# resibots/limbo

Measured on AMD Instinct MI355X. Metric: GP compute()+log_lik evaluations/sec at N=4096 D=6 fp64, higher is better.
Workload: dtype f64

## Files before the change

limbo_amd/csrc/potrf_tail.hip:

```cpp
#include "potrf_tile.h"
#include <array>
#include <map>
#include <mutex>
#include <vector>
#ifdef DIAG_TIMING
__device__ long long g_tail_ts[64][4];
__device__ long long g_tail_cyc[64][4];
#define TTS(c, i) do { if (threadIdx.x == 0 && (c) < 64) { g_tail_ts[(c)][(i)] = wall_clock64(); g_tail_cyc[(c)][(i)] = clock64(); } } while (0)
__device__ long long g_tail_ts2[64][12];
#define TTS2(x, on, i) do { if ((on) && threadIdx.x == 0 && ((x).R0 - (x).p0) / NB < 64) g_tail_ts2[((x).R0 - (x).p0) / NB][(i)] = wall_clock64(); } while (0)
#else
#define TTS(c, i) do { } while (0)
#define TTS2(x, on, i) do { } while (0)
#endif

struct TailArgs {
    double* A;
    int64_t lda, t0;
    int nt, nb;
    int nfull;
    int rhs_rows;
    double* Xt;
    int* info;
    double *LP, *SP, *LPn, *SPn;
    int spin_limit;
    const int* order;
    const double* Xg;
    int64_t ldx, Ns;
    const double* Om;
    int64_t ldom;
    double* Al;
    int64_t ldal;
    int P;
};
#define TAIL_LDS_DOUBLES (4 * NB * PS)
static_assert(TAIL_LDS_DOUBLES >= NB * XS + 3 * NB * PS && TAIL_LDS_DOUBLES * 8 <= 160 * 1024, "k_tail LDS carve");
static __device__ __forceinline__ int tail_tile_id(int nb, int b, int c) { return c * nb - (c * (c - 1)) / 2 + (b - c); }

static __device__ __forceinline__ void tail_gen_tile(const TailArgs& a, const KParams* __restrict__ kp, int64_t I, int64_t J0,
                                                     double (&out)[8])
{
    if (I >= a.Ns) {
        const double* om = a.Om + (I - a.Ns) * a.ldom;
#pragma unroll
        for (int it = 0; it < 8; ++it)
            out[it] = om[J0 + 2 * it];
        return;
    }
    double z[8];
#pragma unroll
    for (int it = 0; it < 8; ++it)
        z[it] = 0.0;
    const int D = kp->D;
    for (int d = 0; d < D; ++d) {
        const double* xr = a.Xg + (int64_t)d * a.ldx;
        const double xi = xr[I], ie = kp->inv_ell[d];
#pragma unroll
        for (int it = 0; it < 8; ++it) {
            const double q = (xi - xr[J0 + 2 * it]) * ie;
            z[it] = fma(q, q, z[it]);
        }
    }
    const int kind = kp->kind;
    const double sf2 = kp->sf2, da = kp->diag_add;
#pragma unroll
    for (int it = 0; it < 8; ++it)
        out[it] = kfun_fast_rt(kind, z[it], sf2) + (I == J0 + 2 * it ? da : 0.0);
}

#define CH_T 10240
#define CH_X11 (CH_T + NB * PS)
#define CH_LD (CH_X11 + 32 * 34)
#define CH_D 0
#define CH_AUX (NB * XS)
#define CH_YS (CH_AUX + 1096)
#define CH_X22 (CH_AUX + 1096 + DIAG_XW_DOUBLES)
static_assert(CH_X22 + 32 * 34 <= CH_T && CH_YS + 32 * PS <= CH_X22 && CH_LD + 32 * 34 <= 4 * NB * PS, "chain workgroup LDS carve");

template <int KLEN>
static __device__ __forceinline__ void syrk40(const double* __restrict__ Aop, int ak0, int wave, int lane, double (&acc)[5])
{
    const int r16 = lane & 15, kq = lane >> 4, c4 = lane & 3;
    const int j1 = wave, j2 = 15 - wave;
    if (wave < 4) {
#pragma unroll
        for (int ks = 0; ks < KLEN; ks += 4) {
            const double* row = Aop + (ak0 + ks + kq) * PS;
            const double a0 = row[r16], a1 = row[16 + r16], a2 = row[32 + r16], a3 = row[48 + r16];
            const double b1 = row[4 * j1 + c4], b2 = row[4 * j2 + c4];
            acc[0] = mfma4(a0, b1, acc[0]);
            acc[1] = mfma4(a1, b1, acc[1]);
            acc[2] = mfma4(a2, b1, acc[2]);
            acc[3] = mfma4(a3, b1, acc[3]);
            acc[4] = mfma4(a3, b2, acc[4]);
        }
    }
    else {
#pragma unroll
        for (int ks = 0; ks < KLEN; ks += 4) {
            const double* row = Aop + (ak0 + ks + kq) * PS;
            const double a1 = row[16 + r16], a2 = row[32 + r16], a3 = row[48 + r16];
            const double b1 = row[4 * j1 + c4], b2 = row[4 * j2 + c4];
            acc[0] = mfma4(a1, b1, acc[0]);
            acc[1] = mfma4(a2, b1, acc[1]);
            acc[2] = mfma4(a3, b1, acc[2]);
            acc[3] = mfma4(a2, b2, acc[3]);
            acc[4] = mfma4(a3, b2, acc[4]);
        }
    }
}
static __host__ __device__ __forceinline__ int tri_solve_cols(int wave)
{
    const int hq = wave >> 1;
    return hq == 0 ? 0 : (hq == 1 ? 8 : (hq == 2 ? 24 : 16));
}
static __device__ __forceinline__ void tri_solve32(const double* __restrict__ Aop, int ak0, const double* __restrict__ X, int wm,
                                                   int hn, int lane, double (&y)[2][2])
{
    const int ar = wm + (lane & 15), bc = hn + (lane & 3), kq = lane >> 4;
#pragma unroll
    for (int ks = 0; ks < 32; ks += 4) {
        if (ks >= hn + 8)
            break;
        double af[2], bf[2];
#pragma unroll
        for (int m = 0; m < 2; ++m)
            af[m] = Aop[(ak0 + ks + kq) * PS + ar + 16 * m];
#pragma unroll
        for (int n = 0; n < 2; ++n)
            bf[n] = X[(bc + 4 * n) * 34 + ks + kq];
#pragma unroll
        for (int n = 0; n < 2; ++n)
#pragma unroll
            for (int m = 0; m < 2; ++m)
                y[m][n] = mfma4(af[m], bf[n], y[m][n]);
    }
}

template <int NW, int STRIDE = 512>
static __device__ __forceinline__ void chain_watch(const unsigned long long* __restrict__ p, unsigned long long (&b)[NW], int spin_limit,
                                                   int* __restrict__ info)
{
    static_assert(NW == 2 || NW == 4, "written out: the words stay in registers");
    const unsigned long long SENT = ~0ull;
    int spins = 0;
    if constexpr (NW == 4) {
        while (b[0] == SENT || b[1] == SENT || b[2] == SENT || b[3] == SENT) {
            if (++spins > spin_limit) {
                info[2] = 1;
                break;
            }
            if (b[0] == SENT) b[0] = __hip_atomic_load(p, __ATOMIC_RELAXED, __HIP_MEMORY_SCOPE_AGENT);
            if (b[1] == SENT) b[1] = __hip_atomic_load(p + STRIDE, __ATOMIC_RELAXED, __HIP_MEMORY_SCOPE_AGENT);
            if (b[2] == SENT) b[2] = __hip_atomic_load(p + 2 * STRIDE, __ATOMIC_RELAXED, __HIP_MEMORY_SCOPE_AGENT);
            if (b[3] == SENT) b[3] = __hip_atomic_load(p + 3 * STRIDE, __ATOMIC_RELAXED, __HIP_MEMORY_SCOPE_AGENT);
        }
    }
    else {
        while (b[0] == SENT || b[1] == SENT) {
            if (++spins > spin_limit) {
                info[2] = 1;
                break;
            }
            if (b[0] == SENT) b[0] = __hip_atomic_load(p, __ATOMIC_RELAXED, __HIP_MEMORY_SCOPE_AGENT);
            if (b[1] == SENT) b[1] = __hip_atomic_load(p + STRIDE, __ATOMIC_RELAXED, __HIP_MEMORY_SCOPE_AGENT);
        }
    }
    asm volatile("" ::: "memory");
}
static __device__ __forceinline__ void chain_watch2(const unsigned long long* __restrict__ pa, unsigned long long (&a)[4],
                                                    const unsigned long long* __restrict__ pb, unsigned long long (&b)[4], int spin_limit,
                                                    int* __restrict__ info)
{
    const unsigned long long SENT = ~0ull;
    constexpr int STRIDE = 8 * NB;
    int spins = 0;
    while (a[0] == SENT || a[1] == SENT || a[2] == SENT || a[3] == SENT || b[0] == SENT || b[1] == SENT || b[2] == SENT || b[3] == SENT) {
        if (++spins > spin_limit) {
            info[2] = 1;
            break;
        }
        if (a[0] == SENT) a[0] = __hip_atomic_load(pa, __ATOMIC_RELAXED, __HIP_MEMORY_SCOPE_AGENT);
        if (a[1] == SENT) a[1] = __hip_atomic_load(pa + STRIDE, __ATOMIC_RELAXED, __HIP_MEMORY_SCOPE_AGENT);
        if (a[2] == SENT) a[2] = __hip_atomic_load(pa + 2 * STRIDE, __ATOMIC_RELAXED, __HIP_MEMORY_SCOPE_AGENT);
        if (a[3] == SENT) a[3] = __hip_atomic_load(pa + 3 * STRIDE, __ATOMIC_RELAXED, __HIP_MEMORY_SCOPE_AGENT);
        if (b[0] == SENT) b[0] = __hip_atomic_load(pb, __ATOMIC_RELAXED, __HIP_MEMORY_SCOPE_AGENT);
        if (b[1] == SENT) b[1] = __hip_atomic_load(pb + STRIDE, __ATOMIC_RELAXED, __HIP_MEMORY_SCOPE_AGENT);
        if (b[2] == SENT) b[2] = __hip_atomic_load(pb + 2 * STRIDE, __ATOMIC_RELAXED, __HIP_MEMORY_SCOPE_AGENT);
        if (b[3] == SENT) b[3] = __hip_atomic_load(pb + 3 * STRIDE, __ATOMIC_RELAXED, __HIP_MEMORY_SCOPE_AGENT);
    }
    asm volatile("" ::: "memory");
}
static __host__ __device__ __forceinline__ void syrk40_units(int wave, int q, int& i, int& j)
{
    if (wave < 4) {
        i = q < 4 ? q : 3;
        j = q < 4 ? wave : 15 - wave;
    }
    else {
        i = q < 3 ? q + 1 : q - 1;
        j = q < 3 ? wave : 15 - wave;
    }
}
static __device__ __forceinline__ void syrk40_load_neg(const double* __restrict__ Dl, int wave, int lane, double (&acc)[5])
{
    const int drow = 4 * ((lane >> 2) & 3) + (lane >> 4), dcol = lane & 3;
#pragma unroll
    for (int q = 0; q < 5; ++q) {
        int i, j;
        syrk40_units(wave, q, i, j);
        acc[q] = -Dl[(16 * i + drow) * XS + 4 * j + dcol];
    }
}
static __device__ __forceinline__ void syrk40_store_neg(double* __restrict__ Dl, int wave, int lane, const double (&acc)[5])
{
    const int drow = 4 * ((lane >> 2) & 3) + (lane >> 4), dcol = lane & 3;
#pragma unroll
    for (int q = 0; q < 5; ++q) {
        int i, j;
        syrk40_units(wave, q, i, j);
        Dl[(16 * i + drow) * XS + 4 * j + dcol] = -acc[q];
    }
}

static __device__ __forceinline__ void tail_chain_updates_and_crossing(const TailArgs& a, const P256& x, double* __restrict__ lds,
                                                                       const int c, const double (&cl)[8], const double (&cv)[8])
{
    const int lane = threadIdx.x & 63, wave = __builtin_amdgcn_readfirstlane(threadIdx.x >> 6);
    const int wm = (wave & 1) * 32, wn = (wave >> 1) * 16;
    const int hn = tri_solve_cols(wave);
    const int crow = wm + (lane & 31), ccol = wn + (lane >> 5);
    const int drow = 4 * ((lane >> 2) & 3) + (lane >> 4), dcol = lane & 3;
    double* const T = lds + CH_T;
    double* const X11 = lds + CH_X11;
    double* const Ld = lds + CH_LD;
    double* const Dl = lds + CH_D;
    double* const Ys = lds + CH_YS;
    double* const X22 = lds + CH_X22;
    const double* Sq = a.SP + (int64_t)(c - 1) * 3072;
    double* pub = a.LP + (int64_t)tail_tile_id(a.nb, c, c - 1) * (NB * NB);
    const unsigned long long* Sp = reinterpret_cast<const unsigned long long*>(Sq) + threadIdx.x;
    double a2v[5];
#pragma unroll
    for (int it = 0; it < 8; ++it)
        lds[crow * XS + ccol + 2 * it] = cv[it];
    __syncthreads();
    syrk40_load_neg(lds, wave, lane, a2v);
    __syncthreads();
    unsigned long long xb[4];
    if (c > 1) {
        PolledTile pa, pb;
        pa.issue(a.LP + (int64_t)tail_tile_id(a.nb, c, 0) * (NB * NB));
        pb.issue(a.LP + (int64_t)tail_tile_id(a.nb, c - 1, 0) * (NB * NB));
        double a2l[2][4] = {{0.0, 0.0, 0.0, 0.0}, {0.0, 0.0, 0.0, 0.0}};
#pragma unroll 1
        for (int s = 0; s < c - 2; ++s) {
            double* const opA = lds + ((c - 2 - s) & 1) * (2 * NB * PS);
            double* const opB = opA + NB * PS;
            pa.finish(a.LP + (int64_t)tail_tile_id(a.nb, c, s) * (NB * NB), x.spin_limit, x.info);
            pa.store(opA);
            pb.finish(a.LP + (int64_t)tail_tile_id(a.nb, c - 1, s) * (NB * NB), x.spin_limit, x.info);
            pb.store(opB);
            pa.issue(a.LP + (int64_t)tail_tile_id(a.nb, c, s + 1) * (NB * NB));
            pb.issue(a.LP + (int64_t)tail_tile_id(a.nb, c - 1, s + 1) * (NB * NB));
            __syncthreads();
            mm64<false>(opA, opB, wm, wn, lane, a2l);
            syrk40<NB>(opA, 0, wave, lane, a2v);
        }
        double* const opA = lds;
        double* const opB = lds + NB * PS;
        {
            const int i = threadIdx.x & 63, kk0 = threadIdx.x >> 6;
            const unsigned long long* ga = reinterpret_cast<const unsigned long long*>(a.LP + (int64_t)tail_tile_id(a.nb, c, c - 2) * (NB * NB)) + i + kk0 * NB;
            const unsigned long long* gb = reinterpret_cast<const unsigned long long*>(a.LP + (int64_t)tail_tile_id(a.nb, c - 1, c - 2) * (NB * NB)) + i + kk0 * NB;
            unsigned long long ha[4] = {pa.b[0], pa.b[1], pa.b[2], pa.b[3]}, hb[4] = {pb.b[0], pb.b[1], pb.b[2], pb.b[3]};
            chain_watch2(ga, ha, gb, hb, x.spin_limit, x.info);
            TTS2(x, true, 8);
#pragma unroll
            for (int q = 0; q < 4; ++q) {
                opA[(kk0 + 8 * q) * PS + i] = __longlong_as_double((long long)ha[q]);
                opB[(kk0 + 8 * q) * PS + i] = __longlong_as_double((long long)hb[q]);
            }
            __syncthreads();
#pragma unroll
            for (int it = 0; it < 8; ++it)
                T[(ccol + 2 * it) * PS + crow] = cl[it];
            mmk<false, 32, 4>(opA, 0, opB, 0, wm, wn, lane, a2l);
            syrk40<32>(opA, 0, wave, lane, a2v);
            unsigned long long ka[4] = {pa.b[4], pa.b[5], pa.b[6], pa.b[7]}, kb[4] = {pb.b[4], pb.b[5], pb.b[6], pb.b[7]};
            chain_watch2(ga + 32 * NB, ka, gb + 32 * NB, kb, x.spin_limit, x.info);
            TTS2(x, true, 9);
#pragma unroll
            for (int q = 0; q < 4; ++q) {
                opA[(32 + kk0 + 8 * q) * PS + i] = __longlong_as_double((long long)ka[q]);
                opB[(32 + kk0 + 8 * q) * PS + i] = __longlong_as_double((long long)kb[q]);
            }
            __syncthreads();
            TTS2(x, true, 10);
            mmk<false, 32, 4>(opA, 32, opB, 32, wm, wn, lane, a2l);
            syrk40<32>(opA, 32, wave, lane, a2v);
#pragma unroll
            for (int q = 0; q < 4; ++q)
                xb[q] = __hip_atomic_load(Sp + 512 * q, __ATOMIC_RELAXED, __HIP_MEMORY_SCOPE_AGENT);
        }
#pragma unroll
        for (int m = 0; m < 2; ++m)
#pragma unroll
            for (int n = 0; n < 4; ++n) {
                double* t = T + (wn + 4 * n + dcol) * PS + wm + 16 * m + drow;
                *t = *t - a2l[m][n];
            }
    }
    else {
#pragma unroll
        for (int it = 0; it < 8; ++it)
            T[(ccol + 2 * it) * PS + crow] = cl[it];
#pragma unroll
        for (int q = 0; q < 4; ++q)
            xb[q] = __hip_atomic_load(Sp + 512 * q, __ATOMIC_RELAXED, POLL_FIRST_SCOPE);
    }
    TTS(c, 0);
    {
        chain_watch<4>(Sp, xb, x.spin_limit, x.info);
        TTS2(x, true, 0);
#pragma unroll
        for (int q = 0; q < 2; ++q) {
            const int e = threadIdx.x + 512 * q;
            X11[(e >> 5) * 34 + (e & 31)] = __longlong_as_double((long long)xb[q]);
            Ld[(e & 31) * 34 + (e >> 5)] = __longlong_as_double((long long)xb[2 + q]);
        }
    }
    __syncthreads();
    diag_flow_init(reinterpret_cast<DiagSync*>(lds + CH_AUX + DIAG_LTB + NB));
    double y1[2][2] = {{0.0, 0.0}, {0.0, 0.0}};
    tri_solve32(T, 0, X11, wm, hn, lane, y1);
#pragma unroll
    for (int m = 0; m < 2; ++m)
#pragma unroll
        for (int n = 0; n < 2; ++n)
            Ys[(hn + 4 * n + dcol) * PS + wm + 16 * m + drow] = y1[m][n];
    __syncthreads();
    TTS2(x, true, 6);
    double u[2][2] = {{0.0, 0.0}, {0.0, 0.0}};
    mmk<true, 32, 2, 34>(Ys, 0, Ld, 0, wm, hn, lane, u);
#pragma unroll
    for (int m = 0; m < 2; ++m)
#pragma unroll
        for (int n = 0; n < 2; ++n) {
            double* t = T + (32 + hn + 4 * n + dcol) * PS + wm + 16 * m + drow;
            *t = *t - u[m][n];
            T[(hn + 4 * n + dcol) * PS + wm + 16 * m + drow] = y1[m][n];
        }
    {
        const int i = threadIdx.x & 63, kk0 = threadIdx.x >> 6;
#pragma unroll
        for (int q = 0; q < 4; ++q) {
            const int col = kk0 + 8 * q;
            __hip_atomic_store(pub + i + NB * col, Ys[col * PS + i], __ATOMIC_RELAXED, __HIP_MEMORY_SCOPE_AGENT);
        }
    }
    TTS2(x, true, 7);
    unsigned long long xc[2];
    xc[0] = __hip_atomic_load(Sp + 2048, __ATOMIC_RELAXED, __HIP_MEMORY_SCOPE_AGENT);
    xc[1] = __hip_atomic_load(Sp + 2048 + 512, __ATOMIC_RELAXED, __HIP_MEMORY_SCOPE_AGENT);
    syrk40<32>(Ys, 0, wave, lane, a2v);
    TTS2(x, true, 1);
    {
        chain_watch<2>(Sp + 2048, xc, x.spin_limit, x.info);
        TTS2(x, true, 2);
        const int e0 = threadIdx.x, e1 = threadIdx.x + 512;
        X22[(e0 >> 5) * 34 + (e0 & 31)] = __longlong_as_double((long long)xc[0]);
        X22[(e1 >> 5) * 34 + (e1 & 31)] = __longlong_as_double((long long)xc[1]);
    }
    __syncthreads();
    TTS2(x, true, 3);
    double y2[2][2] = {{0.0, 0.0}, {0.0, 0.0}};
    tri_solve32(T, 32, X22, wm, hn, lane, y2);
#pragma unroll
    for (int m = 0; m < 2; ++m)
#pragma unroll
        for (int n = 0; n < 2; ++n)
            Ys[(hn + 4 * n + dcol) * PS + wm + 16 * m + drow] = y2[m][n];
    __syncthreads();
    TTS2(x, true, 4);
    syrk40<32>(Ys, 0, wave, lane, a2v);
    syrk40_store_neg(Dl, wave, lane, a2v);
    {
        const int i = threadIdx.x & 63, kk0 = threadIdx.x >> 6;
#pragma unroll
        for (int q = 0; q < 4; ++q) {
            const int col = kk0 + 8 * q;
            __hip_atomic_store(pub + i + NB * (32 + col), Ys[col * PS + i], __ATOMIC_RELAXED, __HIP_MEMORY_SCOPE_AGENT);
        }
    }
#pragma unroll
    for (int m = 0; m < 2; ++m)
#pragma unroll
        for (int n = 0; n < 2; ++n)
            T[(32 + hn + 4 * n + dcol) * PS + wm + 16 * m + drow] = y2[m][n];
    TTS2(x, true, 5);
}

static __device__ __forceinline__ void tail_tile_solve(const P256& x, double* __restrict__ lds, const double (&own)[8],
                                                       const double* __restrict__ Sq, double* __restrict__ pub, const bool near)
{
    const int lane = threadIdx.x & 63, wave = __builtin_amdgcn_readfirstlane(threadIdx.x >> 6);
    const int wm = (wave & 1) * 32, wn = (wave >> 1) * 16;
    const int hn = tri_solve_cols(wave);
    const int crow = wm + (lane & 31), ccol = wn + (lane >> 5);
    const int drow = 4 * ((lane >> 2) & 3) + (lane >> 4), dcol = lane & 3;
    double* const T = lds + CH_T;
    double* const X11 = lds + CH_X11;
    double* const Ld = lds + CH_LD;
    double* const Ys = lds + CH_YS;
    double* const X22 = lds + CH_X22;
    const unsigned long long SENT = ~0ull;
    const unsigned long long* Sp = reinterpret_cast<const unsigned long long*>(Sq) + threadIdx.x;
#pragma unroll
    for (int it = 0; it < 8; ++it)
        T[(ccol + 2 * it) * PS + crow] = own[it];
    {
        unsigned long long xb[4];
#pragma unroll
        for (int q = 0; q < 4; ++q)
            xb[q] = __hip_atomic_load(Sp + 512 * q, __ATOMIC_RELAXED, POLL_FIRST_SCOPE);
        if (near)
            chain_watch<4>(Sp, xb, x.spin_limit, x.info);
        else {
            int spins = 0;
            while (xb[0] == SENT || xb[1] == SENT || xb[2] == SENT || xb[3] == SENT) {
                if (++spins > x.spin_limit) {
                    x.info[2] = 1;
                    break;
                }
                poll_one(Sq + 1023, x.spin_limit, x.info);
                poll_one(Sq + 1024 + 32 * 31, x.spin_limit, x.info);
#pragma unroll
                for (int q = 0; q < 4; ++q)
                    if (xb[q] == SENT)
                        xb[q] = __hip_atomic_load(Sp + 512 * q, __ATOMIC_RELAXED, __HIP_MEMORY_SCOPE_AGENT);
            }
        }
#pragma unroll
        for (int q = 0; q < 2; ++q) {
            const int e = threadIdx.x + 512 * q;
            X11[(e >> 5) * 34 + (e & 31)] = __longlong_as_double((long long)xb[q]);
            Ld[(e & 31) * 34 + (e >> 5)] = __longlong_as_double((long long)xb[2 + q]);
        }
    }
    __syncthreads();
    double y1[2][2] = {{0.0, 0.0}, {0.0, 0.0}};
    tri_solve32(T, 0, X11, wm, hn, lane, y1);
#pragma unroll
    for (int m = 0; m < 2; ++m)
#pragma unroll
        for (int n = 0; n < 2; ++n)
            Ys[(hn + 4 * n + dcol) * PS + wm + 16 * m + drow] = y1[m][n];
    __syncthreads();
    double u[2][2] = {{0.0, 0.0}, {0.0, 0.0}};
    mmk<true, 32, 2, 34>(Ys, 0, Ld, 0, wm, hn, lane, u);
#pragma unroll
    for (int m = 0; m < 2; ++m)
#pragma unroll
        for (int n = 0; n < 2; ++n) {
            double* t = T + (32 + hn + 4 * n + dcol) * PS + wm + 16 * m + drow;
            *t = *t - u[m][n];
            T[(hn + 4 * n + dcol) * PS + wm + 16 * m + drow] = y1[m][n];
        }
    {
        const int i = threadIdx.x & 63, kk0 = threadIdx.x >> 6;
#pragma unroll
        for (int q = 0; q < 4; ++q) {
            const int col = kk0 + 8 * q;
            __hip_atomic_store(pub + i + NB * col, Ys[col * PS + i], __ATOMIC_RELAXED, __HIP_MEMORY_SCOPE_AGENT);
        }
    }
    {
        unsigned long long xc[2];
        xc[0] = __hip_atomic_load(Sp + 2048, __ATOMIC_RELAXED, POLL_FIRST_SCOPE);
        xc[1] = __hip_atomic_load(Sp + 2048 + 512, __ATOMIC_RELAXED, POLL_FIRST_SCOPE);
        if (near)
            chain_watch<2>(Sp + 2048, xc, x.spin_limit, x.info);
        else {
            int spins = 0;
            while (xc[0] == SENT || xc[1] == SENT) {
                if (++spins > x.spin_limit) {
                    x.info[2] = 1;
                    break;
                }
                poll_one(Sq + 2048 + 1023, x.spin_limit, x.info);
                if (xc[0] == SENT)
                    xc[0] = __hip_atomic_load(Sp + 2048, __ATOMIC_RELAXED, __HIP_MEMORY_SCOPE_AGENT);
                if (xc[1] == SENT)
                    xc[1] = __hip_atomic_load(Sp + 2048 + 512, __ATOMIC_RELAXED, __HIP_MEMORY_SCOPE_AGENT);
            }
        }
        const int e0 = threadIdx.x, e1 = threadIdx.x + 512;
        X22[(e0 >> 5) * 34 + (e0 & 31)] = __longlong_as_double((long long)xc[0]);
        X22[(e1 >> 5) * 34 + (e1 & 31)] = __longlong_as_double((long long)xc[1]);
    }
    __syncthreads();
    double y2[2][2] = {{0.0, 0.0}, {0.0, 0.0}};
    tri_solve32(T, 32, X22, wm, hn, lane, y2);
#pragma unroll
    for (int m = 0; m < 2; ++m)
#pragma unroll
        for (int n = 0; n < 2; ++n)
            Ys[(hn + 4 * n + dcol) * PS + wm + 16 * m + drow] = y2[m][n];
    __syncthreads();
    {
        const int i = threadIdx.x & 63, kk0 = threadIdx.x >> 6;
#pragma unroll
        for (int q = 0; q < 4; ++q) {
            const int col = kk0 + 8 * q;
            __hip_atomic_store(pub + i + NB * (32 + col), Ys[col * PS + i], __ATOMIC_RELAXED, __HIP_MEMORY_SCOPE_AGENT);
        }
    }
#pragma unroll
    for (int m = 0; m < 2; ++m)
#pragma unroll
        for (int n = 0; n < 2; ++n)
            T[(32 + hn + 4 * n + dcol) * PS + wm + 16 * m + drow] = y2[m][n];
    __syncthreads();
}

static __device__ __forceinline__ void tail_body(const TailArgs& a, const int wgid, double* __restrict__ lds,
                                                 const KParams* __restrict__ kp = nullptr)
{
    const int lane = threadIdx.x & 63, wave = __builtin_amdgcn_readfirstlane(threadIdx.x >> 6);
    const int wm = (wave & 1) * 32, wn = (wave >> 1) * 16;
    const int crow = wm + (lane & 31), ccol = wn + (lane >> 5);
    int c = 0, b;
    if (a.order) {
        b = __builtin_amdgcn_readfirstlane(a.order[2 * wgid]);
        c = __builtin_amdgcn_readfirstlane(a.order[2 * wgid + 1]);
    }
    else {
        int id = wgid, colh = a.nb;
        while (id >= colh) {
            id -= colh;
            ++c;
            --colh;
        }
        b = c + id;
    }
    const int slot = tail_tile_id(a.nb, b, c);
    const bool mute = a.spin_limit < 0;
    P256 x;
    x.A = a.A;
    x.lda = a.lda;
    x.p0 = a.t0;
    x.R0 = a.t0 + (int64_t)NB * b;
    x.Xt = a.Xt;
    x.info = a.info;
    x.mute = mute;
    x.spin_limit = mute ? -a.spin_limit : a.spin_limit;
    x.nrows = b < a.nfull ? NB : a.rhs_rows;
    x.want_d = false;
    x.Bx = lds;
    x.T0 = lds + NB * XS;
    x.T1 = x.T0 + NB * PS;
    x.T2 = x.T1 + NB * PS;
    x.S22 = a.SP;
    x.HP = a.LP;
    double* const myslot = a.LP + (int64_t)slot * (NB * NB);
    {
        unsigned long long* nx = reinterpret_cast<unsigned long long*>(a.LPn + (int64_t)slot * (NB * NB));
#pragma unroll
        for (int q = 0; q < 8; ++q)
            nx[threadIdx.x + 512 * q] = ~0ull;
        if (b == c) {
            unsigned long long* ns = reinterpret_cast<unsigned long long*>(a.SPn + (int64_t)c * 3072);
#pragma unroll
            for (int q = 0; q < 6; ++q)
                ns[threadIdx.x + 512 * q] = ~0ull;
        }
    }
    if (b == c + 1 && b < a.nt)
        return;
    const int crc = crow < x.nrows ? crow : x.nrows - 1;
    double cv[8];
    if (kp) {
        tail_gen_tile(a, kp, x.R0 + crc, a.t0 + (int64_t)NB * c + ccol, cv);
        if (a.Al && b >= a.nfull && threadIdx.x < NB)
            for (int p = 0; p < a.P; ++p)
                reinterpret_cast<unsigned long long*>(a.Al)[a.t0 + (int64_t)NB * c + threadIdx.x + (int64_t)p * a.ldal] = ~0ull;
    }
    else {
#pragma unroll
        for (int it = 0; it < 8; ++it)
            cv[it] = a.A[x.R0 + crc + (a.t0 + (int64_t)NB * c + ccol + 2 * it) * a.lda];
    }
    if (b == c) {
        double* const Dl = lds + CH_D;
        double* const Ltb = lds + CH_AUX;
        double* const invd = Ltb + DIAG_LTB;
        DiagSync* const sy = reinterpret_cast<DiagSync*>(invd + NB);
        if (c > 0) {
            double cl[8];
            if (kp)
                tail_gen_tile(a, kp, x.R0 + crow, a.t0 + (int64_t)NB * (c - 1) + ccol, cl);
            else {
#pragma unroll
                for (int it = 0; it < 8; ++it)
                    cl[it] = a.A[x.R0 + crow + (a.t0 + (int64_t)NB * (c - 1) + ccol + 2 * it) * a.lda];
            }
            tail_chain_updates_and_crossing(a, x, lds, c, cl, cv);
            TTS(c, 1);
        }
        else {
#pragma unroll
            for (int it = 0; it < 8; ++it)
                Dl[crow * XS + ccol + 2 * it] = cv[it];
            diag_flow_init(sy);
        }
        __syncthreads();
        DiagEarly ea;
        ea.mute = mute;
        ea.S = a.SP + (int64_t)c * 3072;
        TTS(c, 2);
        diag_flow(Dl, Ltb, invd, sy, a.A + x.R0 + x.R0 * a.lda, a.lda, a.Xt + (int64_t)c * (NB * NB), a.info, x.R0, wave, lane,
                  invd + NB + 8, &ea);
        TTS(c, 3);
        if (c > 0) {
            __syncthreads();
            const int i = threadIdx.x & 63, kk0 = threadIdx.x >> 6;
            double* Ag = a.A + x.R0 + (a.t0 + (int64_t)NB * (c - 1)) * a.lda;
            const double* T = lds + CH_T;
#pragma unroll
            for (int q = 0; q < 8; ++q) {
                const int col = kk0 + 8 * q;
                Ag[i + (int64_t)col * a.lda] = T[col * PS + i];
            }
        }
        return;
    }
    PolledTile pa, pb;
    if (c > 0) {
        pa.issue(a.LP + (int64_t)tail_tile_id(a.nb, b, 0) * (NB * NB));
        pb.issue(a.LP + (int64_t)tail_tile_id(a.nb, c, 0) * (NB * NB));
    }
    double a2[2][4] = {{0.0, 0.0, 0.0, 0.0}, {0.0, 0.0, 0.0, 0.0}};
#pragma unroll 1
    for (int s = 0; s < c; ++s) {
        double* const opA = lds + (s & 1) * (2 * NB * PS);
        double* const opB = opA + NB * PS;
        pa.finish(a.LP + (int64_t)tail_tile_id(a.nb, b, s) * (NB * NB), x.spin_limit, x.info);
        pa.store(opA);
        pb.finish(a.LP + (int64_t)tail_tile_id(a.nb, c, s) * (NB * NB), x.spin_limit, x.info);
        pb.store(opB);
        if (s + 1 < c) {
            pa.issue(a.LP + (int64_t)tail_tile_id(a.nb, b, s + 1) * (NB * NB));
            pb.issue(a.LP + (int64_t)tail_tile_id(a.nb, c, s + 1) * (NB * NB));
        }
        __syncthreads();
        mm64<false>(opA, opB, wm, wn, lane, a2);
    }
    if (c > 0) {
        double a2r[8];
        wave_tile_to_rows(a2, a2r, lane);
#pragma unroll
        for (int it = 0; it < 8; ++it)
            cv[it] -= a2r[it];
        __syncthreads();
    }
    tail_tile_solve(x, lds, cv, a.SP + (int64_t)c * 3072, myslot, b - c <= 3);
    {
        const int i = threadIdx.x & 63, kk0 = threadIdx.x >> 6;
        double* Ag = a.A + x.R0 + (a.t0 + (int64_t)NB * c) * a.lda;
        const double* T = lds + CH_T;
        if (i < x.nrows) {
#pragma unroll
            for (int q = 0; q < 8; ++q) {
                const int col = kk0 + 8 * q;
                Ag[i + (int64_t)col * a.lda] = T[col * PS + i];
            }
        }
    }
}

__global__ __launch_bounds__(512) void k_tail(TailArgs a)
{
    __shared__ __attribute__((aligned(16))) double lds[TAIL_LDS_DOUBLES];
    tail_body(a, (int)blockIdx.x, lds);
}
__global__ __launch_bounds__(512) void k_tail_g(TailArgs a, KParams kp)
{
    __shared__ __attribute__((aligned(16))) double lds[TAIL_LDS_DOUBLES];
    tail_body(a, (int)blockIdx.x, lds, &kp);
}
__global__ __launch_bounds__(512) void k_tail_b(TailArgs a, const BatchTab* __restrict__ bt)
{
    __shared__ __attribute__((aligned(16))) double lds[TAIL_LDS_DOUBLES];
    const int G = bt->G, gp = (int)blockIdx.x % G;
    a.A = bt_rebase(bt, gp, a.A);
    a.Xt = bt_rebase(bt, gp, a.Xt);
    a.info = bt_rebase(bt, gp, a.info);
    a.LP = bt_rebase(bt, gp, a.LP);
    a.SP = bt_rebase(bt, gp, a.SP);
    a.LPn = bt_rebase(bt, gp, a.LPn);
    a.SPn = bt_rebase(bt, gp, a.SPn);
    if (a.Xg) {
        a.Xg = bt_rebase(bt, gp, a.Xg);
        a.Om = bt_rebase(bt, gp, a.Om);
        a.Al = bt_rebase(bt, gp, a.Al);
    }
    tail_body(a, (int)blockIdx.x / G, lds, a.Xg ? &bt->kp[gp] : nullptr);
}

__global__ __launch_bounds__(256) void k_ragged_partial(const double* __restrict__ A, int64_t ld, int m, int n, int64_t k, int kc,
                                                        double* __restrict__ part)
{
    __shared__ __attribute__((aligned(16))) double As[32][NB];
    const int li = threadIdx.x & 63, lk = threadIdx.x >> 6;
    const int ti = threadIdx.x & 15, tj = threadIdx.x >> 4;
    const int64_t k0 = (int64_t)blockIdx.x * kc, k1 = k0 + kc < k ? k0 + kc : k;
    double acc[4][4];
#pragma unroll
    for (int r = 0; r < 4; ++r)
#pragma unroll
        for (int c = 0; c < 4; ++c)
            acc[r][c] = 0.0;
    double nx[8];
    auto fetch = [&](int64_t kb) {
#pragma unroll
        for (int q = 0; q < 8; ++q) {
            const int kk = lk + 4 * q;
            nx[q] = (kb + kk < k1 && li < m) ? A[li + (kb + kk) * ld] : 0.0;
        }
    };
    fetch(k0);
    for (int64_t kb = k0; kb < k1; kb += 32) {
        __syncthreads();
#pragma unroll
        for (int q = 0; q < 8; ++q)
            As[lk + 4 * q][li] = nx[q];
        if (kb + 32 < k1)
            fetch(kb + 32);
        __syncthreads();
#pragma unroll 8
        for (int kk = 0; kk < 32; ++kk) {
            double a[4], b[4];
#pragma unroll
            for (int r = 0; r < 4; ++r) {
                a[r] = As[kk][4 * ti + r];
                b[r] = As[kk][4 * tj + r];
            }
#pragma unroll
            for (int r = 0; r < 4; ++r)
#pragma unroll
                for (int c = 0; c < 4; ++c)
                    acc[r][c] = fma(a[r], b[c], acc[r][c]);
        }
    }
    double* out = part + (int64_t)blockIdx.x * (NB * NB);
#pragma unroll
    for (int c = 0; c < 4; ++c)
#pragma unroll
        for (int r = 0; r < 4; ++r)
            out[4 * ti + r + NB * (4 * tj + c)] = acc[r][c];
}
#define RAGGED_MAX_G 32
__global__ __launch_bounds__(256) void k_ragged_fold(double* __restrict__ C, int64_t ldc, int m, int n, int G, const double* __restrict__ part)
{
    const int i = threadIdx.x & 63, j = 4 * (int)blockIdx.x + (threadIdx.x >> 6);
    if (i >= m || j >= n || i < j)
        return;
    double v[RAGGED_MAX_G];
#pragma unroll
    for (int g = 0; g < RAGGED_MAX_G; ++g)
        v[g] = g < G ? part[(int64_t)g * (NB * NB) + i + NB * j] : 0.0;
    double sum = 0.0;
#pragma unroll
    for (int g = 0; g < RAGGED_MAX_G; ++g)
        sum += v[g];
    C[i + (int64_t)j * ldc] -= sum;
}
int ragged_split(int64_t k, int64_t scratch_doubles, int* kc_out)
{
    if (k < 256 || scratch_doubles < 2 * NB * NB)
        return 0;
    int64_t G = k / 64;
    G = G > RAGGED_MAX_G ? RAGGED_MAX_G : G;
    G = G > scratch_doubles / (NB * NB) ? scratch_doubles / (NB * NB) : G;
    const int64_t kc = ((k + G - 1) / G + 31) / 32 * 32;
    G = (k + kc - 1) / kc;
    *kc_out = (int)kc;
    return (int)G;
}
__global__ __launch_bounds__(DIAG_THREADS) void k_ragged_finish(double* __restrict__ C, int64_t ldc, int jb, int P, int G,
                                                                const double* __restrict__ part, double* __restrict__ Lscr,
                                                                double* __restrict__ Xt, int* __restrict__ info, int64_t goff)
{
    __shared__ __attribute__((aligned(16))) double Ls[NB * XS];
    __shared__ __attribute__((aligned(16))) double Ltb[DIAG_LTB];
    __shared__ __attribute__((aligned(16))) double invd[NB];
    __shared__ DiagSync sy;
    __shared__ __attribute__((aligned(16))) double Xw[DIAG_XW_DOUBLES];
    __shared__ double Rr[NB * 65];
    const int lane = threadIdx.x & 63, w = __builtin_amdgcn_readfirstlane(threadIdx.x >> 6);
    const int m = jb + P;
    for (int e = threadIdx.x; e < NB * 65; e += DIAG_THREADS)
        Rr[e] = 0.0;
    for (int e = threadIdx.x; e < NB * NB; e += DIAG_THREADS)
        Ls[(e & 63) * XS + (e >> 6)] = (e & 63) == (e >> 6) ? 1.0 : 0.0;
    __syncthreads();
#pragma unroll 1
    for (int e0 = 0; e0 < NB * jb; e0 += 2 * DIAG_THREADS) {
        double v[2][RAGGED_MAX_G], c0[2];
#pragma unroll
        for (int u = 0; u < 2; ++u) {
            int e = e0 + u * DIAG_THREADS + (int)threadIdx.x;
            e = e < NB * jb ? e : NB * jb - 1;
            const int i = e & 63, j = e >> 6;
#pragma unroll
            for (int g = 0; g < RAGGED_MAX_G; ++g)
                v[u][g] = part[(int64_t)(g < G ? g : G - 1) * (NB * NB) + e];
            c0[u] = C[(i < m ? i : m - 1) + (int64_t)j * ldc];
        }
#pragma unroll
        for (int u = 0; u < 2; ++u) {
            const int e = e0 + u * DIAG_THREADS + (int)threadIdx.x;
            const int i = e & 63, j = e >> 6;
            double sum = 0.0;
#pragma unroll
            for (int g = 0; g < RAGGED_MAX_G; ++g)
                sum += g < G ? v[u][g] : 0.0;
            const double val = c0[u] - sum;
            if (e < NB * jb && i < m && i >= j) {
                if (i < jb)
                    Ls[i * XS + j] = val;
                else
                    Rr[(i - jb) * 65 + j] = val;
            }
        }
    }
    diag_flow_init(&sy);
    __syncthreads();
    diag_flow(Ls, Ltb, invd, &sy, Lscr, NB, Xt, info, goff, w, lane, Xw);
    asm volatile("s_waitcnt vmcnt(0)" ::: "memory");
    __syncthreads();
    for (int e = threadIdx.x; e < NB * NB; e += DIAG_THREADS) {
        const int i = e & 63, j = e >> 6;
        if (i < jb && j <= i)
            C[i + (int64_t)j * ldc] = __hip_atomic_load(Lscr + e, __ATOMIC_RELAXED, __HIP_MEMORY_SCOPE_AGENT);
    }
    if (P > 0) {
        for (int e = threadIdx.x; e < NB * NB; e += DIAG_THREADS)
            Ls[(e >> 6) * XS + (e & 63)] = __hip_atomic_load(Xt + e, __ATOMIC_RELAXED, __HIP_MEMORY_SCOPE_AGENT);
        __syncthreads();
        for (int e = threadIdx.x; e < P * NB; e += DIAG_THREADS) {
            const int c = e & 63, p = e >> 6;
            if (c < jb) {
                double z = 0.0;
                for (int k = 0; k <= c; ++k)
                    z = fma(Rr[p * 65 + k], Ls[c * XS + k], z);
                C[jb + p + (int64_t)c * ldc] = z;
            }
        }
    }
}
bool launch_ragged_finish(hipStream_t s, double* C, int64_t ldc, const double* A, int64_t ld, int64_t jb, int64_t P, int64_t k,
                          double* scratch, int64_t scratch_doubles, double* Xt, int* info, int64_t goff)
{
    const int64_t m = jb + P;
    if (g_batch.bt || g_batch.G != 1 || jb < 1 || jb >= NB || P < 0 || m > NB || !scratch || scratch_doubles < 3 * NB * NB)
        return false;
    int kc = 0;
    const int G = ragged_split(k, scratch_doubles - NB * NB, &kc);
    if (G < 2)
        return false;
    GPE_LAUNCH(k_ragged_partial, dim3((unsigned)G), dim3(256), 0, s, A, ld, (int)m, (int)jb, k, kc, scratch);
    GPE_LAUNCH(k_ragged_finish, dim3(1), dim3(DIAG_THREADS), 0, s, C, ldc, (int)jb, (int)P, G, (const double*)scratch,
               scratch + (int64_t)G * (NB * NB), Xt, info, goff);
    return true;
}
bool launch_ragged_update(hipStream_t s, double* C, int64_t ldc, const double* A, int64_t ld, int64_t m, int64_t n, int64_t k,
                          double* scratch, int64_t scratch_doubles)
{
    if (g_batch.bt || g_batch.G != 1 || m < 1 || m > NB || n < 1 || n > NB || !scratch)
        return false;
    int kc = 0;
    const int G = ragged_split(k, scratch_doubles, &kc);
    if (G < 2)
        return false;
    GPE_LAUNCH(k_ragged_partial, dim3((unsigned)G), dim3(256), 0, s, A, ld, (int)m, (int)n, k, kc, scratch);
    GPE_LAUNCH(k_ragged_fold, dim3(NB / 4), dim3(256), 0, s, C, ldc, (int)m, (int)n, G, (const double*)scratch);
    return true;
}

#define TAIL_DLEAD 4
#define TAIL_DLEAD_MAX_BLOCKED 16
static bool build_tail_order(int nt, int nb, int W, int lag, std::vector<int>& flat, int dlead = 0)
{
    struct T {
        int key, c, b;
    };
    std::vector<T> ts;
    for (int c = 0; c < nt; ++c)
        for (int b = c; b < nb; ++b) {
            int k;
            if (b == c)
                k = 2 * c - 3 - 2 * dlead;
            else if (b >= nt)
                k = 2 * (c + std::max(lag, 0));
            else if (b == c + 1)
                k = 2 * c;
            else
                k = 2 * (W > 0 ? std::max(c, b - W) : c);
            ts.push_back(T{k, c, b});
        }
    std::stable_sort(ts.begin(), ts.end(), [](const T& x, const T& y) {
        if (x.key != y.key)
            return x.key < y.key;
        if (x.c != y.c)
            return x.c < y.c;
        return x.b < y.b;
    });
    auto tid = [&](int b, int c) { return c * nb - (c * (c - 1)) / 2 + (b - c); };
    std::vector<int> pos(ts.size());
    for (size_t i = 0; i < ts.size(); ++i)
        pos[tid(ts[i].b, ts[i].c)] = (int)i;
    auto dpos = [&](int c) { return pos[tid(c, c)]; };
    auto owner = [&](int b, int s) { return (b == s + 1 && b < nt) ? dpos(b) : pos[tid(b, s)]; };
    bool legal = true;
    std::vector<int> blocked(ts.size() + 1, 0);
    for (const T& t : ts) {
        const int me = pos[tid(t.b, t.c)];
        if (t.b == t.c) {
            int last = -1;
            for (int s2 = 0; s2 < t.c - 1; ++s2)
                last = std::max(last, std::max(owner(t.c, s2), owner(t.c - 1, s2)));
            if (last > me) {
                if (dlead <= 0)
                    legal = false;
                ++blocked[(size_t)me + 1];
                --blocked[(size_t)last + 1];
            }
            if (t.c > 0)
                legal = legal && dpos(t.c - 1) < me;
        }
        else if (!(t.b == t.c + 1 && t.b < nt)) {
            for (int s2 = 0; s2 < t.c && legal; ++s2)
                legal = owner(t.b, s2) < me && owner(t.c, s2) < me;
            legal = legal && dpos(t.c) < me;
        }
        if (!legal)
            break;
    }
    for (size_t q = 1, run = 0; q < blocked.size() && legal; ++q) {
        run += blocked[q];
        legal = (int)run <= TAIL_DLEAD_MAX_BLOCKED;
    }
    flat.assign(2 * ts.size(), 0);
    for (size_t i = 0; i < ts.size(); ++i) {
        flat[2 * i] = ts[i].b;
        flat[2 * i + 1] = ts[i].c;
    }
    return legal;
}
static const int* tail_order(int nt, int nb, int dlead, int lag)
{
    const int W = 0;
    if (dlead <= 0 && lag <= 0)
        return nullptr;
    static std::mutex mu;
    static std::map<std::array<int, 6>, int*> cache;
    int dev = 0;
    (void)hipGetDevice(&dev);
    const std::array<int, 6> key{dev, nt, nb, dlead, lag, 0};
    std::lock_guard<std::mutex> lk(mu);
    auto it = cache.find(key);
    if (it != cache.end())
        return it->second;
    std::vector<int> flat;
    int* d = nullptr;
    if (build_tail_order(nt, nb, W, lag, flat, dlead) || (dlead > 0 && build_tail_order(nt, nb, W, lag, flat, 0))) {
        if (hipMalloc(&d, sizeof(int) * flat.size()) != hipSuccess || hipMemcpy(d, flat.data(), sizeof(int) * flat.size(), hipMemcpyHostToDevice) != hipSuccess)
            d = nullptr;
    }
    else
        fprintf(stderr, "gpe: tail_order(%d, %d, lead %d, lag %d) violates a dependency — column-by-column order used\n", nt, nb, dlead, lag);
    cache[key] = d;
    return d;
}
void debug_chain_split(int wave, int* units10, int* cols)
{
    for (int q = 0; q < 5; ++q)
        syrk40_units(wave, q, units10[2 * q], units10[2 * q + 1]);
    *cols = tri_solve_cols(wave);
}
int debug_tail_order(int nt, int nb, int lag, int pair)
{
    if (pair)
        return -1;
    if (nt < 1 || nb < nt || nb > 4096)
        return -1;
    std::vector<int> flat;
    if (!build_tail_order(nt, nb, 0, lag, flat, 0))
        return 0;
    if (!build_tail_order(nt, nb, 0, lag, flat, TAIL_DLEAD))
        return 0;
    std::vector<char> seen((size_t)nt * nb, 0);
    size_t n = 0;
    for (size_t i = 0; i + 1 < flat.size(); i += 2) {
        const int b = flat[i], c = flat[i + 1];
        if (c < 0 || c >= nt || b < c || b >= nb || seen[(size_t)c * nb + b])
            return 0;
        seen[(size_t)c * nb + b] = 1;
        ++n;
    }
    return n == (size_t)(nt * nb - nt * (nt - 1) / 2) ? 1 : 0;
}

void launch_tail(hipStream_t s, double* A, int64_t lda, int64_t t0, int64_t t1, int64_t N64, int64_t M, double* Xt_all, int* info,
                 double* buf_cur, double* buf_next, const TailGen* gen)
{
    TailArgs a{};
    a.A = A;
    a.lda = lda;
    a.t0 = t0;
    a.nt = (int)((t1 - t0) / NB);
    a.nfull = (int)((N64 - t0) / NB);
    a.rhs_rows = (int)(M - N64);
    a.nb = a.nfull + (a.rhs_rows > 0 ? 1 : 0);
    a.Xt = Xt_all + (t0 / NB) * (NB * NB);
    a.info = info;
    a.SP = buf_cur;
    a.LP = buf_cur + (int64_t)a.nt * 3072;
    a.SPn = buf_next;
    a.LPn = buf_next + (int64_t)a.nt * 3072;
    a.spin_limit = flow_spin_limit();
    static const int ord_lag = (int)env_int("GPE_TAIL_LAG", 3);
    a.order = tail_order(a.nt, a.nb, g_batch.bt ? 0 : TAIL_DLEAD, ord_lag);
    const int64_t tiles = tail_tiles(a.nt, a.nb);
    if (gen) {
        a.Xg = gen->Xg;
        a.ldx = gen->ldx;
        a.Ns = gen->Ns;
        a.Om = gen->Om;
        a.ldom = gen->ldom;
        a.Al = gen->Al;
        a.ldal = gen->ldal;
        a.P = gen->P;
    }
    FlowGate gate(s);
    if (g_batch.bt)
        GPE_LAUNCH(k_tail_b, dim3((unsigned)(tiles * g_batch.G)), dim3(512), 0, s, a, g_batch.bt);
    else if (gen)
        GPE_LAUNCH(k_tail_g, dim3((unsigned)tiles), dim3(512), 0, s, a, *gen->kp);
    else
        GPE_LAUNCH(k_tail, dim3((unsigned)tiles), dim3(512), 0, s, a);
}

#ifdef DIAG_TIMING
void dump_tail_timing(int nt)
{
    long long h[64][4];
    hipMemcpyFromSymbol(h, HIP_SYMBOL(g_tail_ts), sizeof(h));
    const long long t0 = h[0][2];
    printf("k_tail, the diagonal workgroups (us after the first one starts factoring): column | earlier updates done | its left tile solved, block complete | factoring | panel wave done\n");
    for (int c = 0; c < nt && c < 64; ++c)
        printf("  %2d | %7.2f | %7.2f | %7.2f | %7.2f   (step %5.2f)\n", c, c ? (h[c][0] - t0) * 0.01 : 0.0, c ? (h[c][1] - t0) * 0.01 : 0.0,
               (h[c][2] - t0) * 0.01, (h[c][3] - t0) * 0.01, c ? (h[c][2] - h[c - 1][2]) * 0.01 : 0.0);
    long long cy[64][4];
    hipMemcpyFromSymbol(cy, HIP_SYMBOL(g_tail_cyc), sizeof(cy));
    printf("  factoring -> panel wave done, per column: us | shader-clock cycles | MHz\n   ");
    for (int c = 0; c < nt && c < 64; ++c)
        printf(" %d: %.2f %lld %.0f |", c, (h[c][3] - h[c][2]) * 0.01, cy[c][3] - cy[c][2], (cy[c][3] - cy[c][2]) / ((h[c][3] - h[c][2]) * 0.01));
    printf("\n");
    long long g[64][12];
    hipMemcpyFromSymbol(g, HIP_SYMBOL(g_tail_ts2), sizeof(g));
    printf("  between two blocks, us after the panel wave of column c-1 is through: X11/L21 seen | phase A done | X22 seen | X22 in LDS | Y2 written | second half product done | block complete | factoring\n");
    for (int c = 1; c < nt && c < 64; ++c) {
        const long long p = h[c - 1][3];
        printf("  %2d | %6.2f | %6.2f | %6.2f | %6.2f | %6.2f | %6.2f | %6.2f | %6.2f   (updates done %6.2f; inside phase A: Y1 in LDS %6.2f, T2 updated + first half out %6.2f)\n", c, (g[c][0] - p) * 0.01, (g[c][1] - p) * 0.01, (g[c][2] - p) * 0.01,
               (g[c][3] - p) * 0.01, (g[c][4] - p) * 0.01, (g[c][5] - p) * 0.01, (h[c][1] - p) * 0.01, (h[c][2] - p) * 0.01, (h[c][0] - p) * 0.01,
               (g[c][6] - p) * 0.01, (g[c][7] - p) * 0.01);
        if (c >= 2)
            printf("       the last update step: first halves of L(c, c-2), L(c-1, c-2) seen %6.2f | second halves seen %6.2f | in LDS %6.2f\n",
                   (g[c][8] - p) * 0.01, (g[c][9] - p) * 0.01, (g[c][10] - p) * 0.01);
    }
}
#endif
```

Measured before the change: 948.9.

## Split tail block's first X11 wait into halves to overlap solve with polling

The diagonal-tile solve in the tail kernel no longer waits for all four published chunks (both X11 halves and L21) at once. It waits for the first X11 half, solves it on the first four waves and starts the syrk product on those rows, then waits for the remaining chunks and solves the second half. The syrk product is split into two 16-row pieces to match, and the final syrk is moved after the second-half publish stores so consumers see data earlier. This adds extra barriers and a variable-arity chain_watch in exchange for overlapping computation with cross-workgroup polling latency.

```diff
diff --git a/limbo_amd/csrc/potrf_tail.hip b/limbo_amd/csrc/potrf_tail.hip
--- a/limbo_amd/csrc/potrf_tail.hip
+++ b/limbo_amd/csrc/potrf_tail.hip
@@ -7,7 +7,7 @@
 __device__ long long g_tail_ts[64][4];
 __device__ long long g_tail_cyc[64][4];
 #define TTS(c, i) do { if (threadIdx.x == 0 && (c) < 64) { g_tail_ts[(c)][(i)] = wall_clock64(); g_tail_cyc[(c)][(i)] = clock64(); } } while (0)
-__device__ long long g_tail_ts2[64][12];
+__device__ long long g_tail_ts2[64][13];
 #define TTS2(x, on, i) do { if ((on) && threadIdx.x == 0 && ((x).R0 - (x).p0) / NB < 64) g_tail_ts2[((x).R0 - (x).p0) / NB][(i)] = wall_clock64(); } while (0)
 #else
 #define TTS(c, i) do { } while (0)
@@ -141,10 +141,30 @@
 static __device__ __forceinline__ void chain_watch(const unsigned long long* __restrict__ p, unsigned long long (&b)[NW], int spin_limit,
                                                    int* __restrict__ info)
 {
-    static_assert(NW == 2 || NW == 4, "written out: the words stay in registers");
+    static_assert(NW >= 1 && NW <= 4, "written out: the words stay in registers");
     const unsigned long long SENT = ~0ull;
     int spins = 0;
-    if constexpr (NW == 4) {
+    if constexpr (NW == 1) {
+        while (b[0] == SENT) {
+            if (++spins > spin_limit) {
+                info[2] = 1;
+                break;
+            }
+            b[0] = __hip_atomic_load(p, __ATOMIC_RELAXED, __HIP_MEMORY_SCOPE_AGENT);
+        }
+    }
+    else if constexpr (NW == 3) {
+        while (b[0] == SENT || b[1] == SENT || b[2] == SENT) {
+            if (++spins > spin_limit) {
+                info[2] = 1;
+                break;
+            }
+            if (b[0] == SENT) b[0] = __hip_atomic_load(p, __ATOMIC_RELAXED, __HIP_MEMORY_SCOPE_AGENT);
+            if (b[1] == SENT) b[1] = __hip_atomic_load(p + STRIDE, __ATOMIC_RELAXED, __HIP_MEMORY_SCOPE_AGENT);
+            if (b[2] == SENT) b[2] = __hip_atomic_load(p + 2 * STRIDE, __ATOMIC_RELAXED, __HIP_MEMORY_SCOPE_AGENT);
+        }
+    }
+    else if constexpr (NW == 4) {
         while (b[0] == SENT || b[1] == SENT || b[2] == SENT || b[3] == SENT) {
             if (++spins > spin_limit) {
                 info[2] = 1;
@@ -320,25 +340,50 @@
             xb[q] = __hip_atomic_load(Sp + 512 * q, __ATOMIC_RELAXED, POLL_FIRST_SCOPE);
     }
     TTS(c, 0);
+    unsigned long long xlo[1] = {xb[0]}, xhi[3] = {xb[1], xb[2], xb[3]};
     {
-        chain_watch<4>(Sp, xb, x.spin_limit, x.info);
+        chain_watch<1>(Sp, xlo, x.spin_limit, x.info);
+        TTS2(x, true, 11);
+        const int e = threadIdx.x;
+        X11[(e >> 5) * 34 + (e & 31)] = __longlong_as_double((long long)xlo[0]);
+    }
+    __syncthreads();
+    diag_flow_init(reinterpret_cast<DiagSync*>(lds + CH_AUX + DIAG_LTB + NB));
+#pragma unroll
+    for (int q = 0; q < 3; ++q)
+        xhi[q] = __hip_atomic_load(Sp + 512 * (q + 1), __ATOMIC_RELAXED, __HIP_MEMORY_SCOPE_AGENT);
+    double y1[2][2] = {{0.0, 0.0}, {0.0, 0.0}};
+    if (wave < 4) {
+        tri_solve32(T, 0, X11, wm, hn, lane, y1);
+#pragma unroll
+        for (int m = 0; m < 2; ++m)
+#pragma unroll
+            for (int n = 0; n < 2; ++n)
+                Ys[(hn + 4 * n + dcol) * PS + wm + 16 * m + drow] = y1[m][n];
+    }
+    __syncthreads();
+    syrk40<16>(Ys, 0, wave, lane, a2v);
+    TTS2(x, true, 12);
+    {
+        chain_watch<3>(Sp + 512, xhi, x.spin_limit, x.info);
         TTS2(x, true, 0);
+        const int e = threadIdx.x + 512;
+        X11[(e >> 5) * 34 + (e & 31)] = __longlong_as_double((long long)xhi[0]);
 #pragma unroll
         for (int q = 0; q < 2; ++q) {
-            const int e = threadIdx.x + 512 * q;
-            X11[(e >> 5) * 34 + (e & 31)] = __longlong_as_double((long long)xb[q]);
-            Ld[(e & 31) * 34 + (e >> 5)] = __longlong_as_double((long long)xb[2 + q]);
-        }
-    }
-    __syncthreads();
-    diag_flow_init(reinterpret_cast<DiagSync*>(lds + CH_AUX + DIAG_LTB + NB));
-    double y1[2][2] = {{0.0, 0.0}, {0.0, 0.0}};
-    tri_solve32(T, 0, X11, wm, hn, lane, y1);
-#pragma unroll
-    for (int m = 0; m < 2; ++m)
-#pragma unroll
-        for (int n = 0; n < 2; ++n)
-            Ys[(hn + 4 * n + dcol) * PS + wm + 16 * m + drow] = y1[m][n];
+            const int el = threadIdx.x + 512 * q;
+            Ld[(el & 31) * 34 + (el >> 5)] = __longlong_as_double((long long)xhi[1 + q]);
+        }
+    }
+    __syncthreads();
+    if (wave >= 4) {
+        tri_solve32(T, 0, X11, wm, hn, lane, y1);
+#pragma unroll
+        for (int m = 0; m < 2; ++m)
+#pragma unroll
+            for (int n = 0; n < 2; ++n)
+                Ys[(hn + 4 * n + dcol) * PS + wm + 16 * m + drow] = y1[m][n];
+    }
     __syncthreads();
     TTS2(x, true, 6);
     double u[2][2] = {{0.0, 0.0}, {0.0, 0.0}};
@@ -363,7 +408,7 @@
     unsigned long long xc[2];
     xc[0] = __hip_atomic_load(Sp + 2048, __ATOMIC_RELAXED, __HIP_MEMORY_SCOPE_AGENT);
     xc[1] = __hip_atomic_load(Sp + 2048 + 512, __ATOMIC_RELAXED, __HIP_MEMORY_SCOPE_AGENT);
-    syrk40<32>(Ys, 0, wave, lane, a2v);
+    syrk40<16>(Ys, 16, wave, lane, a2v);
     TTS2(x, true, 1);
     {
         chain_watch<2>(Sp + 2048, xc, x.spin_limit, x.info);
@@ -383,8 +428,6 @@
             Ys[(hn + 4 * n + dcol) * PS + wm + 16 * m + drow] = y2[m][n];
     __syncthreads();
     TTS2(x, true, 4);
-    syrk40<32>(Ys, 0, wave, lane, a2v);
-    syrk40_store_neg(Dl, wave, lane, a2v);
     {
         const int i = threadIdx.x & 63, kk0 = threadIdx.x >> 6;
 #pragma unroll
@@ -393,6 +436,8 @@
             __hip_atomic_store(pub + i + NB * (32 + col), Ys[col * PS + i], __ATOMIC_RELAXED, __HIP_MEMORY_SCOPE_AGENT);
         }
     }
+    syrk40<32>(Ys, 0, wave, lane, a2v);
+    syrk40_store_neg(Dl, wave, lane, a2v);
 #pragma unroll
     for (int m = 0; m < 2; ++m)
 #pragma unroll
@@ -1069,7 +1114,7 @@
     for (int c = 0; c < nt && c < 64; ++c)
         printf(" %d: %.2f %lld %.0f |", c, (h[c][3] - h[c][2]) * 0.01, cy[c][3] - cy[c][2], (cy[c][3] - cy[c][2]) / ((h[c][3] - h[c][2]) * 0.01));
     printf("\n");
-    long long g[64][12];
+    long long g[64][13];
     hipMemcpyFromSymbol(g, HIP_SYMBOL(g_tail_ts2), sizeof(g));
     printf("  between two blocks, us after the panel wave of column c-1 is through: X11/L21 seen | phase A done | X22 seen | X22 in LDS | Y2 written | second half product done | block complete | factoring\n");
     for (int c = 1; c < nt && c < 64; ++c) {
@@ -1080,6 +1125,7 @@
         if (c >= 2)
             printf("       the last update step: first halves of L(c, c-2), L(c-1, c-2) seen %6.2f | second halves seen %6.2f | in LDS %6.2f\n",
                    (g[c][8] - p) * 0.01, (g[c][9] - p) * 0.01, (g[c][10] - p) * 0.01);
+        printf("       phase A's first row piece: X11 rows 0..15 seen %6.2f | its products done %6.2f\n", (g[c][11] - p) * 0.01, (g[c][12] - p) * 0.01);
     }
 }
 #endif
```

Result: no change. 948.6, median of 3 (-0.0%).
